# FindoraNetwork/ark-bulletproofs

Hardware: AMD Instinct MI355X
Metric: r1cs_constraints_proved_per_sec (+ r1cs_batch_verifies_per_sec under "verify") (higher is better)
Workload: dtype u32x9 (256-bit modular integers, radix 2^29)

## Files before the change

ark_bulletproofs_amd/csrc/ec.cuh:

```cuda
#pragma once
#include "fp29.cuh"

namespace arkbp {

struct Aff {
    Fe x, y;
};
struct Jac {
    Fe X, Y, Z;
};

ARKBP_HD bool aff_is_inf(const Aff& p) { return fe_is_zero_exact(p.x) && fe_is_zero_exact(p.y); }
ARKBP_HD bool jac_is_inf(const Jac& p) { return fe_is_zero_exact(p.Z); }
template <class C> ARKBP_HD Jac jac_inf() {
    Jac r;
    r.X = fe_one<typename C::Fq>();
    r.Y = fe_one<typename C::Fq>();
    r.Z = fe_zero<typename C::Fq>();
    return r;
}
template <class C> ARKBP_HD Jac jac_from_aff(const Aff& p) {
    if (aff_is_inf(p)) return jac_inf<C>();
    Jac r;
    r.X = p.x;
// ... 51 lines not shown
        o.Y = fe_wred<F>(fe_sub<F, 16>(Y3, fe_times<8>(YYYY)));
        o.Z = fe_mul<F>(fe_dbl(p.Y), p.Z);
    }
    return o;
}

template <class C> ARKBP_HD Jac jac_madd(const Jac& p, const Aff& q) {
    typedef typename C::Fq F;
    if (aff_is_inf(q)) return p;
    if (jac_is_inf(p)) {
        Jac r;
        r.X = q.x;
        r.Y = fe_wred<F>(q.y);
        r.Z = fe_one<F>();
        return r;
    }
    Fe Z1Z1 = fe_sqr<F>(p.Z);
    Fe U2 = fe_mul<F>(q.x, Z1Z1);
    Fe S2 = fe_mul<F>(q.y, fe_mul<F>(p.Z, Z1Z1));
    Fe H = fe_sub<F, 4>(U2, p.X);
    Fe r = fe_sub<F, 4>(S2, p.Y);
    if (fe_is_zero_mod<F>(H)) {
        if (fe_is_zero_mod<F>(r)) return jac_dbl<C>(p);
        return jac_inf<C>();
    }
    Fe HH = fe_sqr<F>(H);
    Fe HHH = fe_mul<F>(H, HH);
    Fe V = fe_mul<F>(p.X, HH);
    Jac o;
    o.X = fe_wred<F>(fe_sub<F, 4>(fe_sqr<F>(r), fe_add(HHH, fe_dbl(V))));
    o.Y = fe_mul2<F>(r, fe_sub<F, 4>(V, o.X), fe_neg<F, 4>(p.Y), HHH);
    o.Z = fe_mul<F>(p.Z, H);
    return o;
}

template <class C> ARKBP_HD Jac jac_madd_fast(const Jac& p, const Aff& q, bool& rare) {
    typedef typename C::Fq F;
    Fe Z1Z1 = fe_sqr<F>(p.Z);
    Fe U2 = fe_mul<F>(q.x, Z1Z1);
    Fe S2 = fe_mul<F>(q.y, fe_mul<F>(p.Z, Z1Z1));
    Fe H = fe_sub<F, 4>(U2, p.X);
    Fe r = fe_sub<F, 4>(S2, p.Y);
    rare = aff_is_inf(q) | jac_is_inf(p) | fe_maybe_zero_mod<F>(H);
    Fe HH = fe_sqr<F>(H);
    Fe HHH = fe_mul<F>(H, HH);
    Fe V = fe_mul<F>(p.X, HH);
    Jac o;
    o.X = fe_wred<F>(fe_sub<F, 4>(fe_sqr<F>(r), fe_add(HHH, fe_dbl(V))));
    o.Y = fe_mul2<F>(r, fe_sub<F, 4>(V, o.X), fe_neg<F, 4>(p.Y), HHH);
    o.Z = fe_mul<F>(p.Z, H);
    return o;
}

template <class C> ARKBP_HD Jac jac_add(const Jac& p, const Jac& q) {
    typedef typename C::Fq F;
    if (jac_is_inf(q)) return p;
    if (jac_is_inf(p)) return q;
    Fe Z1Z1 = fe_sqr<F>(p.Z), Z2Z2 = fe_sqr<F>(q.Z);
    Fe U1 = fe_mul<F>(p.X, Z2Z2), U2 = fe_mul<F>(q.X, Z1Z1);
    Fe S1 = fe_mul<F>(p.Y, fe_mul<F>(q.Z, Z2Z2)), S2 = fe_mul<F>(q.Y, fe_mul<F>(p.Z, Z1Z1));
    Fe H = fe_sub<F, 2>(U2, U1);
    Fe r = fe_sub<F, 2>(S2, S1);
    if (fe_is_zero_mod<F>(H)) {
        if (fe_is_zero_mod<F>(r)) return jac_dbl<C>(p);
        return jac_inf<C>();
    }
    Fe HH = fe_sqr<F>(H);
    Fe HHH = fe_mul<F>(H, HH);
    Fe V = fe_mul<F>(U1, HH);
    Jac o;
    o.X = fe_wred<F>(fe_sub<F, 4>(fe_sqr<F>(r), fe_add(HHH, fe_dbl(V))));
    o.Y = fe_mul2<F>(r, fe_sub<F, 4>(V, o.X), fe_neg<F, 2>(S1), HHH);
    o.Z = fe_mul<F>(fe_mul<F>(p.Z, q.Z), H);
    return o;
}

template <class C> ARKBP_HD Aff jac_to_aff_with_zinv(const Jac& p, const Fe& zinv) {
    typedef typename C::Fq F;
    Aff r;
    if (jac_is_inf(p)) {
        r.x = fe_zero<F>();
        r.y = fe_zero<F>();
        return r;
    }
    Fe zi2 = fe_sqr<F>(zinv);
    r.x = fe_canon<F>(fe_mul<F>(p.X, zi2));
    r.y = fe_canon<F>(fe_mul<F>(p.Y, fe_mul<F>(zi2, zinv)));
    return r;
}
template <class C> ARKBP_HD Aff jac_to_aff(const Jac& p) {
    return jac_to_aff_with_zinv<C>(p, fe_inv<typename C::Fq>(p.Z));
}

template <class F> ARKBP_DEV_NOINLINE bool fe_sqrt(Fe& out, const Fe& a_in) {
    const Fe a = fe_wred<F>(a_in);
    if (fe_is_zero_mod<F>(a)) { out = fe_zero<F>(); return true; }
    const Fe a2 = fe_sqr<F>(a), a3 = fe_mul<F>(a2, a);
    Fe w = fe_one<F>();
#pragma unroll 1
    for (int wd = 7; wd >= 0; wd--) {
        const u32 e = F::TS_TM1H[wd];
#pragma unroll 1
        for (int bit = 30; bit >= 0; bit -= 2) {
            w = fe_sqr<F>(fe_sqr<F>(w));
            const u32 d = (e >> bit) & 3u;
            if (d) {
// ... 83 lines not shown
```

ark_bulletproofs_amd/csrc/fp29.cuh:

```cuda
#pragma once
#include <cstdint>
#if defined(__HIPCC__)
#include <hip/hip_runtime.h>
#define ARKBP_HD __host__ __device__ __forceinline__
#define ARKBP_DEV_NOINLINE __device__ __noinline__
#else
#define ARKBP_HD inline
#define ARKBP_DEV_NOINLINE inline
#endif
#include "arkbp_params.h"

#ifdef ARKBP_CHECK_BOUNDS
#include <cstdio>
#include <cstdlib>
#define ARKBP_ASSERT(c, msg) do { if (!(c)) { fprintf(stderr, "fp29 bound violated: %s (%s:%d)\n", msg, __FILE__, __LINE__); abort(); } } while (0)
#else
#define ARKBP_ASSERT(c, msg)
#endif

namespace arkbp {

typedef uint32_t u32;
typedef uint64_t u64;
typedef int32_t i32;
// ... 61 lines not shown
    static_assert(K == 2 || K == 4 || K == 8 || K == 16, "K");
    Fe r;
#pragma unroll
    for (int i = 0; i < 9; i++) {
        const u32 off = K == 2 ? P::SUBK2[i] : K == 4 ? P::SUBK4[i] : K == 8 ? P::SUBK8[i] : P::SUBK16[i];
        ARKBP_ASSERT(i == 8 || a.l[i] <= (2u << 29), "fe_sub: L(a) > 2");
        ARKBP_ASSERT(b.l[i] <= off, "fe_sub: limb of b exceeds the K*p offset");
        r.l[i] = a.l[i] + off - b.l[i];
    }
    return fe_norm(r);
}
template <class P, int K> ARKBP_HD Fe fe_neg(const Fe& a) { return fe_sub<P, K>(fe_zero<P>(), a); }

template <class P, class Col> ARKBP_HD Fe fe_pm_product(Col&& col) {
    static_assert(P::PM, "pseudo-Mersenne fields only");
    constexpr u32 c0 = P::PM_C0, c1 = P::PM_C1;
    u32 H[9];
    u64 acc = 0;
#pragma unroll
    for (int k = 9; k < 17; k++) {
        col(k, acc);
        H[k - 9] = (u32)acc & M29;
        acc >>= 29;
    }
    ARKBP_ASSERT(acc < (1ull << 32), "fe_pm_product: product exceeds 18 limbs");
    H[8] = (u32)acc;
    Fe r;
    acc = 0;
#pragma unroll
    for (int k = 0; k < 9; k++) {
        col(k, acc);
        acc += (u64)H[k] * c0;
        if (c1 != 0 && k > 0) acc += (u64)H[k - 1] * c1;
        r.l[k] = (u32)acc & M29;
        acc >>= 29;
    }
    if (c1 != 0) acc += (u64)H[8] * c1;
    const u64 o1 = acc;
    ARKBP_ASSERT(o1 < (1ull << 41), "fe_pm_product: overflow too large");
    constexpr int sh = P::BITS - 232;
    const u64 o = (o1 << (261 - P::BITS)) + (r.l[8] >> sh);
    r.l[8] &= (1u << sh) - 1u;
    acc = (u64)r.l[0] + o * P::PM_D0;
    r.l[0] = (u32)acc & M29; acc >>= 29;
    acc += (u64)r.l[1] + o * P::PM_D1;
    r.l[1] = (u32)acc & M29; acc >>= 29;
    u32 cy = (u32)acc;
#pragma unroll
    for (int j = 2; j < 8; j++) { const u32 t = r.l[j] + cy; r.l[j] = t & M29; cy = t >> 29; }
    r.l[8] += cy;
    return r;
}

template <class P> ARKBP_HD Fe fe_mul(const Fe& a, const Fe& b) {
#ifdef ARKBP_CHECK_BOUNDS
    { u64 la = 0, lb = 0; for (int i = 0; i < 9; i++) { if (a.l[i] > la) la = a.l[i]; if (b.l[i] > lb) lb = b.l[i]; }
      ARKBP_ASSERT((unsigned __int128)la * lb <= ((unsigned __int128)6 << 58) + ((unsigned __int128)1 << 40), "fe_mul: L(a)*L(b) > 6"); }
#endif
    if constexpr (P::PM) {
        return fe_pm_product<P>([&](int k, u64& acc) {
#pragma unroll
            for (int i = (k < 9 ? 0 : k - 8); i <= (k < 9 ? k : 8); i++) acc += (u64)a.l[i] * b.l[k - i];
        });
    }
    u32 m[9];
    Fe t;
    u64 acc = 0;
#pragma unroll
    for (int k = 0; k < 9; k++) {
#pragma unroll
        for (int i = 0; i <= k; i++) acc += (u64)a.l[i] * b.l[k - i];
#pragma unroll
        for (int i = 0; i < k; i++) acc += (u64)m[i] * P::P29[k - i];
        m[k] = ((u32)acc * P::NINV29) & M29;
        acc += (u64)m[k] * P::P29[0];
        acc >>= 29;
    }
#pragma unroll
    for (int k = 9; k < 17; k++) {
#pragma unroll
        for (int i = k - 8; i < 9; i++) acc += (u64)a.l[i] * b.l[k - i];
#pragma unroll
        for (int i = k - 8; i < 9; i++) acc += (u64)m[i] * P::P29[k - i];
        t.l[k - 9] = (u32)acc & M29;
        acc >>= 29;
    }
    ARKBP_ASSERT(acc < (1ull << 29), "fe_mul: result exceeds 2^261");
    t.l[8] = (u32)acc;
    return t;
}

template <class P> ARKBP_HD Fe fe_mul2(const Fe& a, const Fe& b, const Fe& c, const Fe& d) {
#ifdef ARKBP_CHECK_BOUNDS
    { u64 la = 0, lb = 0, lc = 0, ld = 0;
      for (int i = 0; i < 9; i++) { if (a.l[i] > la) la = a.l[i]; if (b.l[i] > lb) lb = b.l[i]; if (c.l[i] > lc) lc = c.l[i]; if (d.l[i] > ld) ld = d.l[i]; }
      ARKBP_ASSERT((unsigned __int128)la * lb + (unsigned __int128)lc * ld <= ((unsigned __int128)6 << 58) + ((unsigned __int128)1 << 41), "fe_mul2: L(a)*L(b) + L(c)*L(d) > 6"); }
#endif
    if constexpr (P::PM) {
        return fe_pm_product<P>([&](int k, u64& acc) {
#pragma unroll
            for (int i = (k < 9 ? 0 : k - 8); i <= (k < 9 ? k : 8); i++) { acc += (u64)a.l[i] * b.l[k - i]; acc += (u64)c.l[i] * d.l[k - i]; }
        });
    }
    u32 m[9];
    Fe t;
    u64 acc = 0;
#pragma unroll
    for (int k = 0; k < 9; k++) {
#pragma unroll
        for (int i = 0; i <= k; i++) { acc += (u64)a.l[i] * b.l[k - i]; acc += (u64)c.l[i] * d.l[k - i]; }
#pragma unroll
        for (int i = 0; i < k; i++) acc += (u64)m[i] * P::P29[k - i];
        m[k] = ((u32)acc * P::NINV29) & M29;
        acc += (u64)m[k] * P::P29[0];
        acc >>= 29;
    }
#pragma unroll
    for (int k = 9; k < 17; k++) {
#pragma unroll
        for (int i = k - 8; i < 9; i++) { acc += (u64)a.l[i] * b.l[k - i]; acc += (u64)c.l[i] * d.l[k - i]; }
#pragma unroll
        for (int i = k - 8; i < 9; i++) acc += (u64)m[i] * P::P29[k - i];
        t.l[k - 9] = (u32)acc & M29;
        acc >>= 29;
    }
    ARKBP_ASSERT(acc < (1ull << 29), "fe_mul2: result exceeds 2^261");
    t.l[8] = (u32)acc;
    return t;
}

template <class P> ARKBP_HD Fe fe_sqr(const Fe& a) {
    u32 m[9], a2[9];
#pragma unroll
    for (int i = 0; i < 9; i++) a2[i] = a.l[i] << 1;
#ifdef ARKBP_CHECK_BOUNDS
    for (int i = 0; i < 9; i++) ARKBP_ASSERT(a.l[i] <= (2u << 29) + 16, "fe_sqr: L(a) > 2");
#endif
    if constexpr (P::PM) {
        return fe_pm_product<P>([&](int k, u64& acc) {
#pragma unroll
            for (int i = (k < 9 ? 0 : k - 8); 2 * i < k; i++) acc += (u64)a2[i] * a.l[k - i];
            if ((k & 1) == 0) acc += (u64)a.l[k / 2] * a.l[k / 2];
        });
    }
    Fe t;
    u64 acc = 0;
#pragma unroll
    for (int k = 0; k < 9; k++) {
#pragma unroll
        for (int i = 0; 2 * i < k; i++) acc += (u64)a2[i] * a.l[k - i];
        if ((k & 1) == 0) acc += (u64)a.l[k / 2] * a.l[k / 2];
#pragma unroll
        for (int i = 0; i < k; i++) acc += (u64)m[i] * P::P29[k - i];
        m[k] = ((u32)acc * P::NINV29) & M29;
        acc += (u64)m[k] * P::P29[0];
        acc >>= 29;
    }
#pragma unroll
    for (int k = 9; k < 17; k++) {
#pragma unroll
        for (int i = k - 8; 2 * i < k; i++) acc += (u64)a2[i] * a.l[k - i];
        if ((k & 1) == 0) acc += (u64)a.l[k / 2] * a.l[k / 2];
#pragma unroll
        for (int i = k - 8; i < 9; i++) acc += (u64)m[i] * P::P29[k - i];
        t.l[k - 9] = (u32)acc & M29;
        acc >>= 29;
    }
    t.l[8] = (u32)acc;
    return t;
}

template <class P> ARKBP_HD Fe fe_wred(const Fe& a) {
    if constexpr (P::PM) {
        constexpr int shp = P::BITS - 232;
        ARKBP_ASSERT(a.l[8] < (1u << 29) + 8u, "fe_wred: a >= 2^261");
        const u32 o = a.l[8] >> shp;
        Fe r;
        u32 t = a.l[0] + o * P::PM_D0;
        r.l[0] = t & M29;
        t = a.l[1] + o * P::PM_D1 + (t >> 29);
        r.l[1] = t & M29;
        u32 cy = t >> 29;
#pragma unroll
        for (int j = 2; j < 8; j++) { t = a.l[j] + cy; r.l[j] = t & M29; cy = t >> 29; }
        r.l[8] = (a.l[8] & ((1u << shp) - 1u)) + cy;
        return r;
    }
    constexpr int sh = P::WR_BITS - 232;
    u32 q = a.l[8] >> sh;
    if (P::WR_SIGN > 0) q = q ? q - 1 : 0;
    Fe r;
    i64 acc = 0;
#pragma unroll
    for (int i = 0; i < 9; i++) {
        acc += (i64)a.l[i] - (i64)((u64)q * P::P29[i]);
        r.l[i] = (u32)acc & M29;
        acc >>= 29;
    }
    ARKBP_ASSERT(acc == 0, "fe_wred: went negative or overflowed");
    return r;
}

template <class P> ARKBP_HD Fe fe_canon(const Fe& a) {
    Fe w = fe_wred<P>(a);
#pragma unroll
    for (int rep = 0; rep < 2; rep++) {
        Fe d;
        i32 c = 0;
#pragma unroll
        for (int i = 0; i < 9; i++) {
            i32 t = (i32)w.l[i] - (i32)P::P29[i] + c;
            d.l[i] = (u32)t & M29;
            c = t >> 29;
        }
        const bool neg = c < 0;
#pragma unroll
        for (int i = 0; i < 9; i++) w.l[i] = neg ? w.l[i] : d.l[i];
// ... 80 lines not shown
```

ark_bulletproofs_amd/csrc/ipa.cuh:

```cuda
#pragma once
#include "msm.cuh"

namespace arkbp {

template <class F> __global__ void k_scalars_import(const u32* __restrict__ in, u32* __restrict__ out, u32 n) {
    const u32 i = blockIdx.x * blockDim.x + threadIdx.x;
    if (i >= n) return;
    u32 w[8];
    load_words8(w, in + (size_t)i * 8);
    store_fe_dev<F>(out + (size_t)i * 8, fe_load_ark<F>(w));
}
template <class F> __global__ void k_scalars_export(const u32* __restrict__ in, u32* __restrict__ out, u32 n) {
    const u32 i = blockIdx.x * blockDim.x + threadIdx.x;
    if (i >= n) return;
    u32 w[8];
    fe_store_ark<F>(w, load_fe_dev<F>(in + (size_t)i * 8));
    store_words8(out + (size_t)i * 8, w);
}

static constexpr int IMPORT_MAX = 5;
struct ImportList {
    u32* dst[IMPORT_MAX];
    u32 cnt[IMPORT_MAX];
    int nseg;
// ... 443 lines not shown
        u32 w[16];
        aff_store_dev(w, o);
        store_words8(out + ((size_t)e * n + i) * 16, w);
        store_words8(out + ((size_t)e * n + i) * 16 + 8, w + 8);
    }
}
template <class C> __device__ __forceinline__ bool jac_equals_aff(const Jac& J, const Aff& A) {
    typedef typename C::Fq F;
    const bool ji = jac_is_inf(J), ai = aff_is_inf(A);
    if (ji || ai) return ji && ai;
    const Fe zz = fe_sqr<F>(J.Z);
    if (!fe_eq_mod<F>(fe_wred<F>(J.X), fe_mul<F>(A.x, zz))) return false;
    return fe_eq_mod<F>(fe_wred<F>(J.Y), fe_mul<F>(A.y, fe_mul<F>(zz, J.Z)));
}
template <class C> __global__ void __launch_bounds__(256)
k_ftab_check(const u32* __restrict__ gens, const u32* __restrict__ T, u32 n, u32 E, u32 nwin, unsigned long long* __restrict__ bad,
             u32 g_first = 0, u32 g_stride = 1 ) {
    const u32 i = blockIdx.x * blockDim.x + threadIdx.x;
    if (i >= n) return;
    u32 wrong = 0;
    Aff first = load_aff_dev(gens + ((size_t)g_first + (size_t)i * g_stride) * 16);
    Jac expect = jac_from_aff<C>(first);
#pragma unroll 1
    for (u32 j = 0; j < nwin; j++) {
        const u32* row = T + ((size_t)j * E) * n * 16;
        const Aff base = load_aff_dev(row + (size_t)i * 16);
        if (!jac_equals_aff<C>(expect, base)) wrong++;
        Aff prev = base;
#pragma unroll 1
        for (u32 e = 2; e <= E; e++) {
            const Aff cur = load_aff_dev(row + ((size_t)(e - 1) * n + i) * 16);
            if (!jac_equals_aff<C>(jac_madd<C>(jac_from_aff<C>(prev), base), cur)) wrong++;
            prev = cur;
        }
        expect = jac_dbl<C>(jac_from_aff<C>(prev));
    }
    if (wrong) atomicAdd(bad, (unsigned long long)wrong);
}
template <class C> __global__ void __launch_bounds__(256)
k_fb_rows_check(const u32* __restrict__ gens, const u32* __restrict__ T, u32 n, size_t row_points, u32 R, unsigned long long* __restrict__ bad) {
    const u32 i = blockIdx.x * blockDim.x + threadIdx.x;
    if (i >= n) return;
    u32 wrong = 0;
    Jac expect = jac_from_aff<C>(load_aff_dev(gens + (size_t)i * 16));
#pragma unroll 1
    for (u32 r = 0; r < R; r++) {
        const Aff cur = load_aff_dev(T + ((size_t)r * row_points + i) * 16);
        if (!jac_equals_aff<C>(expect, cur)) wrong++;
        expect = jac_dbl<C>(jac_dbl<C>(jac_dbl<C>(jac_dbl<C>(jac_from_aff<C>(cur)))));
    }
    if (wrong) atomicAdd(bad, (unsigned long long)wrong);
}

template <class C> __device__ __forceinline__ Jac ftab_step(Jac acc, const u32* __restrict__ T, u32 n_tab, u32 E, u32 gi, u32 j, u32 e1, u32 e2, bool neg1, bool neg2) {
    typedef typename C::Fq F;
#pragma unroll 1
    for (int h = 0; h < (C::HAS_GLV ? 2 : 1); h++) {
        const u32 e = h ? e2 : e1;
        if (!e) continue;
        const u32* src = T + (((size_t)j * E + (e - 1)) * n_tab + gi) * 16;
        const bool neg = h ? neg2 : neg1;
        Aff P = load_aff_dev(src);
        if constexpr (C::HAS_GLV) { if (h && !aff_is_inf(P)) P.x = fe_mul<F>(P.x, fe_const<F, C::BETA29>()); }
        bool rare;
        Jac nxt = jac_madd_fast<C>(acc, aff_cneg_lazy<C>(P, neg), rare);
        if (__builtin_expect(rare, 0)) {
            Aff Q = load_aff_dev(src);
            if constexpr (C::HAS_GLV) { if (h && !aff_is_inf(Q)) Q.x = fe_mul<F>(Q.x, fe_const<F, C::BETA29>()); }
            nxt = jac_madd<C>(acc, aff_cneg_lazy<C>(Q, neg));
        }
        acc = nxt;
    }
    return acc;
}
template <class C> __global__ void __launch_bounds__(256) __attribute__((amdgpu_waves_per_eu(3)))
k_ipa_fold_tab(const u32* __restrict__ TG, const u32* __restrict__ TH, u32 n_tab, u32 E, u32* __restrict__ G, u32* __restrict__ H, u32 n, FtabDigits dG,
               FtabDigits dH, int which, u32 g_first, u32 g_stride, u32* __restrict__ jac_ws,
               const u32* __restrict__ Gin ,
               const u32* __restrict__ Hin) {
    typedef typename C::Fq F;
    const u32 t = blockIdx.x * blockDim.x + threadIdx.x;
    if (t >= (which == 3 ? 2 * n : n)) return;
    const bool isH = which == 2 || (which == 3 && t >= n);
    const u32 i = (which == 3 && isH) ? t - n : t;
    u32* V = isH ? H : G;
    const u32* T = isH ? TH : TG;
    const u32 gi = g_first + i * g_stride;
    Jac acc = jac_inf<C>();
    const u32 nwin = isH ? dH.nwin : dG.nwin;
#pragma unroll 1
    for (u32 j = 0; j < nwin; j++) {
        const u32 e1 = isH ? dH.e1[j] : dG.e1[j], e2 = isH ? dH.e2[j] : dG.e2[j];
        acc = ftab_step<C>(acc, T, n_tab, E, gi, j, e1, e2, (((isH ? dH.neg1 : dG.neg1) >> j) & 1ull) != 0, (((isH ? dH.neg2 : dG.neg2) >> j) & 1ull) != 0);
    }
    const u32* Vin = isH ? (Hin ? Hin : H) : (Gin ? Gin : G);
    acc = jac_madd<C>(acc, load_aff_dev(Vin + (size_t)(n + i) * 16));
    fold_emit<C>(V, i, t, acc, jac_ws);
}

struct FtabDigits3 {
    FtabDigits d[3];
};
template <class C> __global__ void __launch_bounds__(256) __attribute__((amdgpu_waves_per_eu(3)))
k_ipa_fold_tab2(const u32* __restrict__ TG, const u32* __restrict__ TH, u32 n_tab, u32 E, u32* __restrict__ G, u32* __restrict__ H, u32 m, FtabDigits3 dG,
                FtabDigits3 dH, u32* __restrict__ jac_ws, const u32* __restrict__ Gin, const u32* __restrict__ Hin,
                u32 g_first , u32 g_stride) {
    typedef typename C::Fq F;
    const u32 t = blockIdx.x * blockDim.x + threadIdx.x;
    if (t >= 2 * m) return;
    const bool isH = t >= m;
    const u32 i = isH ? t - m : t;
    const u32 n = 2 * m;
    const u32* T = isH ? TH : TG;
    Jac acc = jac_inf<C>();
#pragma unroll 1
    for (u32 mu = 0; mu < 3; mu++) {
        const u32 gi = g_first + (mu == 0 ? m + i : mu == 1 ? n + i : i) * g_stride;
        const u32 nwin = isH ? dH.d[mu].nwin : dG.d[mu].nwin;
        const unsigned long long neg1 = isH ? dH.d[mu].neg1 : dG.d[mu].neg1, neg2 = isH ? dH.d[mu].neg2 : dG.d[mu].neg2;
#pragma unroll 1
        for (u32 j = 0; j < nwin; j++) {
            const u32 e1 = isH ? dH.d[mu].e1[j] : dG.d[mu].e1[j], e2 = isH ? dH.d[mu].e2[j] : dG.d[mu].e2[j];
            acc = ftab_step<C>(acc, T, n_tab, E, gi, j, e1, e2, ((neg1 >> j) & 1ull) != 0, ((neg2 >> j) & 1ull) != 0);
        }
    }
    acc = jac_madd<C>(acc, load_aff_dev((isH ? Hin : Gin) + (size_t)(n + m + i) * 16));
    fold_emit<C>(isH ? H : G, i, t, acc, jac_ws);
}

}
```

ark_bulletproofs_amd/csrc/msm.cuh:

```cuda
#pragma once
#include "ec.cuh"
#include "fe_io.cuh"
#include "ecq.cuh"
#include "glv.cuh"

namespace arkbp {

#ifndef ARKBP_MSM_CH
#define ARKBP_MSM_CH 16
#endif
static constexpr int MSM_CH = ARKBP_MSM_CH;
static constexpr int MSM_CHL = MSM_CH == 8 ? 3 : MSM_CH == 16 ? 4 : MSM_CH == 32 ? 5 : 6;
static_assert((1 << MSM_CHL) == MSM_CH, "ARKBP_MSM_CH must be 8, 16, 32 or 64");
static constexpr int MSM_CHL_BINNED = MSM_CHL;
static constexpr int MSM_MAXLVL = 8;
static constexpr int MSM_MAXSEG = 6;

struct BaseSegs {
    const u32* ptr[MSM_MAXSEG];
    u32 start[MSM_MAXSEG + 1];
    int nseg;
    u32 fixed_c4;
    u32 tbits;
    u64 row_words[MSM_MAXSEG];
// ... 452 lines not shown
    for (u32 j = 0; j < 8; j++) {
        const u32 b = base + j;
        if (b >= B) break;
        u32 v = cnt[j];
        for (int k = 0; k < nl; k++) { lvl_off[(size_t)k * (B + 1) + b] = excl[k]; excl[k] += v; v = msm_next_level(v, k, chl, b >= b_gen, spl); }
    }
}

__global__ void __launch_bounds__(256) k_msm_scatter(const u32* __restrict__ canon, u32* __restrict__ cursor, u32* __restrict__ entries, MsmPlan pl) {
    const u32 i = blockIdx.x * blockDim.x + threadIdx.x;
    const bool live = i < pl.n;
    u32 k[8];
#pragma unroll
    for (int j = 0; j < 8; j++) k[j] = 0;
    if (live) load_words8(k, canon + (size_t)i * 8);
    u32 carry = 0;
    for (int w = 0; w < pl.W; w++) {
        const int d = msm_digit(k, w, pl.c, carry);
        const bool valid = live && d != 0 && w >= pl.w_lo && w < pl.w_hi;
        const u32 pos = wave_count(cursor, (u32)w * pl.NB + (u32)(d < 0 ? -d : d) - 1, valid);
        if (valid) entries[pos] = (i << 1) | (d < 0 ? 1u : 0u);
    }
}

__device__ __forceinline__ u32 find_bucket(const u32* __restrict__ off, u32 B, u32 j) {
    u32 lo = 0, hi = B;
    while (hi - lo > 1) {
        u32 mid = (lo + hi) >> 1;
        if (off[mid] <= j) lo = mid; else hi = mid;
    }
    return lo;
}

template <class C> __global__ void __launch_bounds__(256)
k_msm_accum(BaseSegs segs, const u32* __restrict__ entries, const u32* __restrict__ off0, const u32* __restrict__ off1, u32* __restrict__ out,
            u32 B, u32 nchunks, int slotted, SlotPlan sp, u32 NB, const u32* __restrict__ boff, int chl) {
    const u32 j = blockIdx.x * blockDim.x + threadIdx.x;
    if (j >= nchunks) return;
    const u32 b = find_bucket(off1, B, j);
    u32 beg, end;
    const u32 r = j - off1[b], k = off1[b + 1] - off1[b];
    u32 s0, cnt;
    if (slotted == 2) {
        s0 = boff[b]; cnt = off0[b + 1] - off0[b];
    } else if (slotted) {
        const u32 w = b / NB, v = b - w * NB;
        s0 = sp.base[w] + v * sp.cap[w]; cnt = off0[b + 1] - off0[b];
    } else {
        s0 = off0[b]; cnt = off0[b + 1] - off0[b];
    }
    const u32 per = k > 1 ? (cnt + k - 1) / k : (1u << chl);
    beg = s0 + min(r * per, cnt);
    end = min(beg + per, s0 + cnt);
    Jac acc = jac_inf<C>();
    if (beg < end) {
        u32 ent = entries[beg];
        u32 ent_n = beg + 1 < end ? entries[beg + 1] : 0u;
        Raw16 raw = load_raw16(seg_base_ptr(segs, ent >> 1));
        for (u32 e = beg; e < end; e++) {
            Raw16 raw_n = raw;
            u32 ent_nn = 0;
            if (e + 1 < end) raw_n = load_raw16(seg_base_ptr(segs, ent_n >> 1));
            if (e + 2 < end) ent_nn = entries[e + 2];
            const Aff p = aff_from_raw(raw);
            if (e == beg) {
                acc = jac_from_aff<C>(aff_cneg_lazy<C>(p, ent & 1));
                acc.Y = fe_wred<typename C::Fq>(acc.Y);
            } else {
                bool rare;
                Jac nxt = jac_madd_fast<C>(acc, aff_cneg_lazy<C>(p, ent & 1), rare);
                if (__builtin_expect(rare, 0)) nxt = jac_madd<C>(acc, aff_cneg_lazy<C>(load_aff_dev(seg_base_ptr(segs, ent >> 1)), ent & 1));
                acc = nxt;
            }
            ent = ent_n; ent_n = ent_nn;
            raw = raw_n;
        }
    }
    store_jac_ws<C>(out + (size_t)j * 24, acc);
}

template <class C> __global__ void __launch_bounds__(256)
k_msm_accum_wave(BaseSegs segs, const u32* __restrict__ entries, const u32* __restrict__ off0, const u32* __restrict__ off_last, u32* __restrict__ out, u32 B,
                 int slotted, SlotPlan sp, u32 NB, const u32* __restrict__ boff) {
    __shared__ u32 sh[4][64 * 27];
    const u32 wv = threadIdx.x >> 6, lane = threadIdx.x & 63;
    const u32 b = blockIdx.x * 4 + wv;
    if (b >= B) return;
    const u32 cnt = off0[b + 1] - off0[b];
    if (!cnt) return;
    u32 beg;
    if (slotted == 2) beg = boff[b];
    else if (slotted) { const u32 w = b / NB, v = b - w * NB; beg = sp.base[w] + v * sp.cap[w]; }
    else beg = off0[b];
    Jac acc = jac_inf<C>();
    for (u32 e = lane; e < cnt; e += 64) {
        const u32 ent = entries[beg + e];
        acc = jac_madd<C>(acc, aff_cneg_lazy<C>(load_aff_dev(seg_base_ptr(segs, ent >> 1)), ent & 1));
    }
    u32* s = sh[wv];
    for (u32 stride = 32; stride >= 1; stride >>= 1) {
        if (lane >= stride && lane < 2 * stride) {
#pragma unroll
            for (int i = 0; i < 9; i++) { s[i * 64 + lane] = acc.X.l[i]; s[(9 + i) * 64 + lane] = acc.Y.l[i]; s[(18 + i) * 64 + lane] = acc.Z.l[i]; }
        }
        __builtin_amdgcn_wave_barrier();
        __threadfence_block();
        if (lane < stride) {
            Jac o;
#pragma unroll
            for (int i = 0; i < 9; i++) { o.X.l[i] = s[i * 64 + lane + stride]; o.Y.l[i] = s[(9 + i) * 64 + lane + stride]; o.Z.l[i] = s[(18 + i) * 64 + lane + stride]; }
            acc = jac_add<C>(acc, o);
        }
        __builtin_amdgcn_wave_barrier();
        __threadfence_block();
    }
    if (lane == 0) store_jac_ws<C>(out + (size_t)off_last[b] * 24, acc);
}

template <class C> __global__ void __launch_bounds__(256)
k_msm_reduce(const u32* __restrict__ in, const u32* __restrict__ off_prev, const u32* __restrict__ off_cur, u32* __restrict__ out, u32 B,
             u32 nchunks, int chl, u32 skip_from ) {
    const u32 j = blockIdx.x * blockDim.x + threadIdx.x;
    if (j >= nchunks) return;
    const u32 b = find_bucket(off_cur, B, j);
    if (b >= skip_from) return;
    const u32 beg = off_prev[b] + ((j - off_cur[b]) << chl);
    const u32 end = min(beg + (1u << chl), off_prev[b + 1]);
    Jac acc = load_jac_ws(in + (size_t)beg * 24);
    for (u32 e = beg + 1; e < end; e++) acc = jac_add<C>(acc, load_jac_ws(in + (size_t)e * 24));
    store_jac_ws<C>(out + (size_t)j * 24, acc);
}
// ... 237 lines not shown
        if ((int)lane >= o) { incl += t2; inclc += t3; }
    }
    if (lane == 63) { wsum[wv] = incl; wsum[4 + wv] = inclc; }
    __syncthreads();
    u32 excl = incl - run, exclc = inclc - runc;
    for (u32 q = 0; q < wv; q++) { excl += wsum[q]; exclc += wsum[4 + q]; }
    const u32 b0 = w * pl.NB + (bin << bp.LB);
    for (u32 x = tid * per; x < min((tid + 1) * per, NF); x++) {
        const u32 cn = cnt[x];
        bcnt[b0 + x] = cn;
        boff[b0 + x] = (u32)region + excl;
        loff[b0 + x] = exclc;
        cnt[x] = excl;
        excl += cn;
        exclc += (cn + chm) / chcap;
    }
    if (tid == 255) bin_chunks[w * bp.NBIN + bin] = exclc;
    if (big > MSM_FS_BUCKET_MAX) *overflow = 1u;
    __syncthreads();
    for (u32 x = tid; x < n; x += 256) {
        const u32 e = buf[x];
        const u32 pos = atomicAdd(&cnt[(e >> 1) & fmask], 1u);
        ent[region + pos] = ((e >> (bp.LB + 1)) << 1) | (e & 1u);
    }
}
__device__ __forceinline__ void fs_bin_range(u32 x, const MsmPlan& pl, const BinPlan& bp, u32& b0, u32& nb) {
    if (x < bp.wb * bp.NBIN) { const u32 w = x / bp.NBIN, bin = x - w * bp.NBIN; b0 = w * (u32)pl.NB + (bin << bp.LB); nb = 1u << bp.LB; }
    else { b0 = ((u32)pl.W - 1u) * (u32)pl.NB; nb = bp.top_nb; }
}
template <class C> __global__ void __launch_bounds__(256)
k_msm_accum_fs(BaseSegs segs, const u32* __restrict__ entries, const u32* __restrict__ bcnt, const u32* __restrict__ loff, const u32* __restrict__ boff,
               const u32* __restrict__ bin_chunks, u32* __restrict__ out, MsmPlan pl, BinPlan bp, FsPlan fp, u32 chcap, u32* __restrict__ info) {
    __shared__ u32 base[MSM_FS_MAXBINS + 1];
    __shared__ u32 ws[4];
    fs_block_scan(bin_chunks, fp.nbins, base, ws);
    const u32 total = min(base[fp.nbins], fp.max_chunks);
    if (blockIdx.x == 0 && threadIdx.x == 0) { info[0] = base[fp.nbins]; info[1] = base[fp.nbins - 1]; }
    const u32 j = blockIdx.x * 256u + threadIdx.x;
    if (j >= total) return;
    u32 lo = 0, hi = fp.nbins;
    while (hi - lo > 1) { const u32 mid = (lo + hi) >> 1; if (base[mid] <= j) lo = mid; else hi = mid; }
    const u32 jj = j - base[lo];
    u32 b0, nb;
    fs_bin_range(lo, pl, bp, b0, nb);
    u32 l2 = 0, h2 = nb;
    while (h2 - l2 > 1) { const u32 mid = (l2 + h2) >> 1; if (loff[b0 + mid] <= jj) l2 = mid; else h2 = mid; }
    const u32 b = b0 + l2;
    const u32 s0 = boff[b];
    const u32 cnt = bcnt[b], r = jj - loff[b];
    const u32 k = (cnt + chcap - 1u) / chcap;
    const u32 per = k > 1 ? (cnt + k - 1) / k : chcap;
    const u32 beg = s0 + min(r * per, cnt);
    const u32 end = min(beg + per, s0 + cnt);
    Jac acc = jac_inf<C>();
    if (beg < end) {
        u32 ent = entries[beg];
        u32 ent_n = beg + 1 < end ? entries[beg + 1] : 0u;
        Raw16 raw = load_raw16(seg_base_ptr(segs, ent >> 1));
        for (u32 e = beg; e < end; e++) {
            Raw16 raw_n = raw;
            u32 ent_nn = 0;
            if (e + 1 < end) raw_n = load_raw16(seg_base_ptr(segs, ent_n >> 1));
            if (e + 2 < end) ent_nn = entries[e + 2];
            Aff p = aff_from_raw(raw);
            if constexpr (C::HAS_GLV) {
                if (segs.glv && (ent & 2u) && !aff_is_inf(p)) p.x = fe_mul<typename C::Fq>(p.x, fe_const<typename C::Fq, C::BETA29>());
            }
            if (e == beg) {
                acc = jac_from_aff<C>(aff_cneg_lazy<C>(p, ent & 1));
                acc.Y = fe_wred<typename C::Fq>(acc.Y);
            } else {
                bool rare;
                Jac nxt = jac_madd_fast<C>(acc, aff_cneg_lazy<C>(p, ent & 1), rare);
                if (__builtin_expect(rare, 0)) {
                    Aff q = load_aff_dev(seg_base_ptr(segs, ent >> 1));
                    if constexpr (C::HAS_GLV) {
                        if (segs.glv && (ent & 2u) && !aff_is_inf(q)) q.x = fe_mul<typename C::Fq>(q.x, fe_const<typename C::Fq, C::BETA29>());
                    }
                    nxt = jac_madd<C>(acc, aff_cneg_lazy<C>(q, ent & 1));
                }
                acc = nxt;
            }
            ent = ent_n; ent_n = ent_nn;
            raw = raw_n;
        }
    }
    store_jac_ws<C>(out + (size_t)j * 24, acc);
}
template <class C, bool QUAD = false> __global__ void __launch_bounds__(256)
k_msm_reduce_fs(const u32* __restrict__ part, const u32* __restrict__ bcnt, const u32* __restrict__ loff, const u32* __restrict__ bin_chunks,
                u32* __restrict__ sums, MsmPlan pl, BinPlan bp, FsPlan fp, u32 chcap, u32 G) {
    __shared__ u32 base[MSM_FS_MAXBINS + 1];
    __shared__ u32 ws[4];
    fs_block_scan(bin_chunks, fp.nbins, base, ws);
    const u32 g = blockIdx.x * 256u + threadIdx.x;
    const u32 nbk = bp.wb * (u32)pl.NB;
    const u32 gb = G == 4 ? g >> 2 : g;
    const u32 b = min(gb, nbk - 1u), q = G == 4 ? g & 3u : 0u;
    const u32 w = b / (u32)pl.NB, v = b - w * (u32)pl.NB;
    const u32 first = base[w * bp.NBIN + (v >> bp.LB)] + loff[b];
    u32 nch = min((bcnt[b] + chcap - 1u) / chcap, MSM_FS_BUCKET_MAX / 8u);
    if (first + nch > fp.max_chunks) nch = 0;
    if (QUAD) {
        Jac acc = jac_inf<C>();
        if (nch) acc = load_jac_ws(part + (size_t)first * 24);
#pragma unroll 1
        for (u32 e = 1; e < nch; e++) acc = qjac_add<C>(acc, load_jac_ws(part + (size_t)(first + e) * 24), q);
        if (q == 0 && gb < nbk) store_jac_ws<C>(sums + (size_t)b * 24, acc);
        return;
    }
    Jac acc = jac_inf<C>();
    u32 e = q;
    int o = 0;
#pragma unroll 1
    while (o >= 0) {
        Jac other;
        bool doit;
        if (o == 0) {
            doit = e < nch;
            if (!__any(doit)) { o = G == 4 ? 2 : -1; continue; }
            if (doit) other = load_jac_ws(part + (size_t)(first + e) * 24);
            e += G;
        } else {
            other = jac_shfl_down(acc, o, 4);
            doit = (int)q < o && q + (u32)o < nch;
            o = o == 2 ? 1 : -1;
        }
        if (doit) acc = jac_add<C>(acc, other);
    }
    if (q == 0 && gb < nbk) store_jac_ws<C>(sums + (size_t)b * 24, acc);
}
template <class C> __device__ __forceinline__ void store_T_ark(u32* __restrict__ o, const Jac& acc) {
    typedef typename C::Fq F;
    u32 wd[8];
    const bool inf = jac_is_inf(acc);
    fe_store_ark<F>(wd, acc.X); store_words8(o, wd);
    fe_store_ark<F>(wd, acc.Y); store_words8(o + 8, wd);
    if (inf) { for (int i = 0; i < 8; i++) wd[i] = 0; } else fe_store_ark<F>(wd, acc.Z);
    store_words8(o + 16, wd);
}
// ... 119 lines not shown
```

Before: 16.83 million.

## Use XYZZ coordinates for bucket and table accumulation; exploit all-ones modulus limbs

Replaces Jacobian accumulators with XYZZ coordinates in the MSM bucket-accumulate kernels and the fixed-table fold steps. Mixed addition then needs about 8 multiplies instead of about 11, and the result is converted back to Jacobian once at the end. Separately, the Montgomery reduction columns group modulus limbs equal to 2^29-1 so their products are summed first and multiplied once, cutting multiplies for moduli with such limbs. The risks are more live registers from the extra coordinate, which may cut occupancy, and slower rare paths that go through conversions.

```diff
diff --git a/ark_bulletproofs_amd/csrc/ec.cuh b/ark_bulletproofs_amd/csrc/ec.cuh
--- a/ark_bulletproofs_amd/csrc/ec.cuh
+++ b/ark_bulletproofs_amd/csrc/ec.cuh
@@ -127,6 +127,66 @@
     return o;
 }
 
+struct Xyzz {
+    Fe X, Y, ZZ, ZZZ;
+};
+ARKBP_HD bool xyzz_is_inf(const Xyzz& p) { return fe_is_zero_exact(p.ZZ); }
+template <class C> ARKBP_HD Xyzz xyzz_inf() {
+    Xyzz r;
+    r.X = fe_one<typename C::Fq>();
+    r.Y = fe_one<typename C::Fq>();
+    r.ZZ = fe_zero<typename C::Fq>();
+    r.ZZZ = fe_zero<typename C::Fq>();
+    return r;
+}
+template <class C> ARKBP_HD Xyzz xyzz_from_aff(const Aff& q) {
+    typedef typename C::Fq F;
+    if (aff_is_inf(q)) return xyzz_inf<C>();
+    Xyzz r;
+    r.X = q.x;
+    r.Y = fe_wred<F>(q.y);
+    r.ZZ = fe_one<F>();
+    r.ZZZ = fe_one<F>();
+    return r;
+}
+template <class C> ARKBP_HD Xyzz xyzz_from_jac(const Jac& p) {
+    typedef typename C::Fq F;
+    Xyzz r;
+    r.X = p.X;
+    r.Y = p.Y;
+    r.ZZ = fe_sqr<F>(p.Z);
+    r.ZZZ = fe_mul<F>(p.Z, r.ZZ);
+    return r;
+}
+template <class C> ARKBP_HD Jac xyzz_to_jac(const Xyzz& p) {
+    typedef typename C::Fq F;
+    Jac r;
+    r.X = fe_mul<F>(p.X, p.ZZ);
+    r.Y = fe_mul<F>(p.Y, p.ZZZ);
+    r.Z = p.ZZ;
+    return r;
+}
+template <class C> ARKBP_HD Xyzz xyzz_madd_fast(const Xyzz& p, const Aff& q, bool& rare) {
+    typedef typename C::Fq F;
+    Fe U2 = fe_mul<F>(q.x, p.ZZ);
+    Fe S2 = fe_mul<F>(q.y, p.ZZZ);
+    Fe H = fe_sub<F, 4>(U2, p.X);
+    Fe r = fe_sub<F, 4>(S2, p.Y);
+    rare = aff_is_inf(q) | xyzz_is_inf(p) | fe_maybe_zero_mod<F>(H);
+    Fe HH = fe_sqr<F>(H);
+    Fe HHH = fe_mul<F>(H, HH);
+    Fe V = fe_mul<F>(p.X, HH);
+    Xyzz o;
+    o.X = fe_wred<F>(fe_sub<F, 4>(fe_sqr<F>(r), fe_add(HHH, fe_dbl(V))));
+    o.Y = fe_mul2<F>(r, fe_sub<F, 4>(V, o.X), fe_neg<F, 4>(p.Y), HHH);
+    o.ZZ = fe_mul<F>(p.ZZ, HH);
+    o.ZZZ = fe_mul<F>(p.ZZZ, HHH);
+    return o;
+}
+template <class C> ARKBP_HD Xyzz xyzz_madd(const Xyzz& p, const Aff& q) {
+    return xyzz_from_jac<C>(jac_madd<C>(xyzz_to_jac<C>(p), q));
+}
+
 template <class C> ARKBP_HD Jac jac_add(const Jac& p, const Jac& q) {
     typedef typename C::Fq F;
     if (jac_is_inf(q)) return p;
diff --git a/ark_bulletproofs_amd/csrc/fp29.cuh b/ark_bulletproofs_amd/csrc/fp29.cuh
--- a/ark_bulletproofs_amd/csrc/fp29.cuh
+++ b/ark_bulletproofs_amd/csrc/fp29.cuh
@@ -137,6 +137,23 @@
     return r;
 }
 
+template <class P> constexpr int fe_ones_limbs() {
+    int n = 0;
+    for (int i = 0; i < 9; i++) n += P::P29[i] == M29 ? 1 : 0;
+    return n;
+}
+template <class P> ARKBP_HD void fe_red_col(u64& acc, const u32 (&m)[9], int k, int lo, int hi) {
+    static_assert(fe_ones_limbs<P>() <= 7, "the sum of the m[i] under all-ones limbs must fit 32 bits");
+    u32 ones = 0;
+    bool any = false;
+#pragma unroll
+    for (int i = lo; i < hi; i++) {
+        if (P::P29[k - i] == M29) { ones += m[i]; any = true; }
+        else acc += (u64)m[i] * P::P29[k - i];
+    }
+    if (any) acc += (u64)ones * M29;
+}
+
 template <class P> ARKBP_HD Fe fe_mul(const Fe& a, const Fe& b) {
 #ifdef ARKBP_CHECK_BOUNDS
     { u64 la = 0, lb = 0; for (int i = 0; i < 9; i++) { if (a.l[i] > la) la = a.l[i]; if (b.l[i] > lb) lb = b.l[i]; }
@@ -155,8 +172,7 @@
     for (int k = 0; k < 9; k++) {
 #pragma unroll
         for (int i = 0; i <= k; i++) acc += (u64)a.l[i] * b.l[k - i];
-#pragma unroll
-        for (int i = 0; i < k; i++) acc += (u64)m[i] * P::P29[k - i];
+        fe_red_col<P>(acc, m, k, 0, k);
         m[k] = ((u32)acc * P::NINV29) & M29;
         acc += (u64)m[k] * P::P29[0];
         acc >>= 29;
@@ -165,8 +181,7 @@
     for (int k = 9; k < 17; k++) {
 #pragma unroll
         for (int i = k - 8; i < 9; i++) acc += (u64)a.l[i] * b.l[k - i];
-#pragma unroll
-        for (int i = k - 8; i < 9; i++) acc += (u64)m[i] * P::P29[k - i];
+        fe_red_col<P>(acc, m, k, k - 8, 9);
         t.l[k - 9] = (u32)acc & M29;
         acc >>= 29;
     }
@@ -194,8 +209,7 @@
     for (int k = 0; k < 9; k++) {
 #pragma unroll
         for (int i = 0; i <= k; i++) { acc += (u64)a.l[i] * b.l[k - i]; acc += (u64)c.l[i] * d.l[k - i]; }
-#pragma unroll
-        for (int i = 0; i < k; i++) acc += (u64)m[i] * P::P29[k - i];
+        fe_red_col<P>(acc, m, k, 0, k);
         m[k] = ((u32)acc * P::NINV29) & M29;
         acc += (u64)m[k] * P::P29[0];
         acc >>= 29;
@@ -204,8 +218,7 @@
     for (int k = 9; k < 17; k++) {
 #pragma unroll
         for (int i = k - 8; i < 9; i++) { acc += (u64)a.l[i] * b.l[k - i]; acc += (u64)c.l[i] * d.l[k - i]; }
-#pragma unroll
-        for (int i = k - 8; i < 9; i++) acc += (u64)m[i] * P::P29[k - i];
+        fe_red_col<P>(acc, m, k, k - 8, 9);
         t.l[k - 9] = (u32)acc & M29;
         acc >>= 29;
     }
@@ -235,8 +248,7 @@
 #pragma unroll
         for (int i = 0; 2 * i < k; i++) acc += (u64)a2[i] * a.l[k - i];
         if ((k & 1) == 0) acc += (u64)a.l[k / 2] * a.l[k / 2];
-#pragma unroll
-        for (int i = 0; i < k; i++) acc += (u64)m[i] * P::P29[k - i];
+        fe_red_col<P>(acc, m, k, 0, k);
         m[k] = ((u32)acc * P::NINV29) & M29;
         acc += (u64)m[k] * P::P29[0];
         acc >>= 29;
@@ -246,8 +258,7 @@
 #pragma unroll
         for (int i = k - 8; 2 * i < k; i++) acc += (u64)a2[i] * a.l[k - i];
         if ((k & 1) == 0) acc += (u64)a.l[k / 2] * a.l[k / 2];
-#pragma unroll
-        for (int i = k - 8; i < 9; i++) acc += (u64)m[i] * P::P29[k - i];
+        fe_red_col<P>(acc, m, k, k - 8, 9);
         t.l[k - 9] = (u32)acc & M29;
         acc >>= 29;
     }
diff --git a/ark_bulletproofs_amd/csrc/ipa.cuh b/ark_bulletproofs_amd/csrc/ipa.cuh
--- a/ark_bulletproofs_amd/csrc/ipa.cuh
+++ b/ark_bulletproofs_amd/csrc/ipa.cuh
@@ -519,7 +519,7 @@
     if (wrong) atomicAdd(bad, (unsigned long long)wrong);
 }
 
-template <class C> __device__ __forceinline__ Jac ftab_step(Jac acc, const u32* __restrict__ T, u32 n_tab, u32 E, u32 gi, u32 j, u32 e1, u32 e2, bool neg1, bool neg2) {
+template <class C> __device__ __forceinline__ Xyzz ftab_step(Xyzz acc, const u32* __restrict__ T, u32 n_tab, u32 E, u32 gi, u32 j, u32 e1, u32 e2, bool neg1, bool neg2) {
     typedef typename C::Fq F;
 #pragma unroll 1
     for (int h = 0; h < (C::HAS_GLV ? 2 : 1); h++) {
@@ -530,11 +530,11 @@
         Aff P = load_aff_dev(src);
         if constexpr (C::HAS_GLV) { if (h && !aff_is_inf(P)) P.x = fe_mul<F>(P.x, fe_const<F, C::BETA29>()); }
         bool rare;
-        Jac nxt = jac_madd_fast<C>(acc, aff_cneg_lazy<C>(P, neg), rare);
+        Xyzz nxt = xyzz_madd_fast<C>(acc, aff_cneg_lazy<C>(P, neg), rare);
         if (__builtin_expect(rare, 0)) {
             Aff Q = load_aff_dev(src);
             if constexpr (C::HAS_GLV) { if (h && !aff_is_inf(Q)) Q.x = fe_mul<F>(Q.x, fe_const<F, C::BETA29>()); }
-            nxt = jac_madd<C>(acc, aff_cneg_lazy<C>(Q, neg));
+            nxt = xyzz_madd<C>(acc, aff_cneg_lazy<C>(Q, neg));
         }
         acc = nxt;
     }
@@ -553,7 +553,7 @@
     u32* V = isH ? H : G;
     const u32* T = isH ? TH : TG;
     const u32 gi = g_first + i * g_stride;
-    Jac acc = jac_inf<C>();
+    Xyzz acc = xyzz_inf<C>();
     const u32 nwin = isH ? dH.nwin : dG.nwin;
 #pragma unroll 1
     for (u32 j = 0; j < nwin; j++) {
@@ -561,8 +561,7 @@
         acc = ftab_step<C>(acc, T, n_tab, E, gi, j, e1, e2, (((isH ? dH.neg1 : dG.neg1) >> j) & 1ull) != 0, (((isH ? dH.neg2 : dG.neg2) >> j) & 1ull) != 0);
     }
     const u32* Vin = isH ? (Hin ? Hin : H) : (Gin ? Gin : G);
-    acc = jac_madd<C>(acc, load_aff_dev(Vin + (size_t)(n + i) * 16));
-    fold_emit<C>(V, i, t, acc, jac_ws);
+    fold_emit<C>(V, i, t, jac_madd<C>(xyzz_to_jac<C>(acc), load_aff_dev(Vin + (size_t)(n + i) * 16)), jac_ws);
 }
 
 struct FtabDigits3 {
@@ -579,7 +578,7 @@
     const u32 i = isH ? t - m : t;
     const u32 n = 2 * m;
     const u32* T = isH ? TH : TG;
-    Jac acc = jac_inf<C>();
+    Xyzz acc = xyzz_inf<C>();
 #pragma unroll 1
     for (u32 mu = 0; mu < 3; mu++) {
         const u32 gi = g_first + (mu == 0 ? m + i : mu == 1 ? n + i : i) * g_stride;
@@ -591,8 +590,7 @@
             acc = ftab_step<C>(acc, T, n_tab, E, gi, j, e1, e2, ((neg1 >> j) & 1ull) != 0, ((neg2 >> j) & 1ull) != 0);
         }
     }
-    acc = jac_madd<C>(acc, load_aff_dev((isH ? Hin : Gin) + (size_t)(n + m + i) * 16));
-    fold_emit<C>(isH ? H : G, i, t, acc, jac_ws);
-}
-
-}
+    fold_emit<C>(isH ? H : G, i, t, jac_madd<C>(xyzz_to_jac<C>(acc), load_aff_dev((isH ? Hin : Gin) + (size_t)(n + m + i) * 16)), jac_ws);
+}
+
+}
diff --git a/ark_bulletproofs_amd/csrc/msm.cuh b/ark_bulletproofs_amd/csrc/msm.cuh
--- a/ark_bulletproofs_amd/csrc/msm.cuh
+++ b/ark_bulletproofs_amd/csrc/msm.cuh
@@ -528,7 +528,7 @@
     const u32 per = k > 1 ? (cnt + k - 1) / k : (1u << chl);
     beg = s0 + min(r * per, cnt);
     end = min(beg + per, s0 + cnt);
-    Jac acc = jac_inf<C>();
+    Xyzz acc = xyzz_inf<C>();
     if (beg < end) {
         u32 ent = entries[beg];
         u32 ent_n = beg + 1 < end ? entries[beg + 1] : 0u;
@@ -540,19 +540,18 @@
             if (e + 2 < end) ent_nn = entries[e + 2];
             const Aff p = aff_from_raw(raw);
             if (e == beg) {
-                acc = jac_from_aff<C>(aff_cneg_lazy<C>(p, ent & 1));
-                acc.Y = fe_wred<typename C::Fq>(acc.Y);
+                acc = xyzz_from_aff<C>(aff_cneg_lazy<C>(p, ent & 1));
             } else {
                 bool rare;
-                Jac nxt = jac_madd_fast<C>(acc, aff_cneg_lazy<C>(p, ent & 1), rare);
-                if (__builtin_expect(rare, 0)) nxt = jac_madd<C>(acc, aff_cneg_lazy<C>(load_aff_dev(seg_base_ptr(segs, ent >> 1)), ent & 1));
+                Xyzz nxt = xyzz_madd_fast<C>(acc, aff_cneg_lazy<C>(p, ent & 1), rare);
+                if (__builtin_expect(rare, 0)) nxt = xyzz_madd<C>(acc, aff_cneg_lazy<C>(load_aff_dev(seg_base_ptr(segs, ent >> 1)), ent & 1));
                 acc = nxt;
             }
             ent = ent_n; ent_n = ent_nn;
             raw = raw_n;
         }
     }
-    store_jac_ws<C>(out + (size_t)j * 24, acc);
+    store_jac_ws<C>(out + (size_t)j * 24, xyzz_to_jac<C>(acc));
 }
 
 template <class C> __global__ void __launch_bounds__(256)
@@ -896,7 +895,7 @@
     const u32 per = k > 1 ? (cnt + k - 1) / k : chcap;
     const u32 beg = s0 + min(r * per, cnt);
     const u32 end = min(beg + per, s0 + cnt);
-    Jac acc = jac_inf<C>();
+    Xyzz acc = xyzz_inf<C>();
     if (beg < end) {
         u32 ent = entries[beg];
         u32 ent_n = beg + 1 < end ? entries[beg + 1] : 0u;
@@ -911,17 +910,16 @@
                 if (segs.glv && (ent & 2u) && !aff_is_inf(p)) p.x = fe_mul<typename C::Fq>(p.x, fe_const<typename C::Fq, C::BETA29>());
             }
             if (e == beg) {
-                acc = jac_from_aff<C>(aff_cneg_lazy<C>(p, ent & 1));
-                acc.Y = fe_wred<typename C::Fq>(acc.Y);
+                acc = xyzz_from_aff<C>(aff_cneg_lazy<C>(p, ent & 1));
             } else {
                 bool rare;
-                Jac nxt = jac_madd_fast<C>(acc, aff_cneg_lazy<C>(p, ent & 1), rare);
+                Xyzz nxt = xyzz_madd_fast<C>(acc, aff_cneg_lazy<C>(p, ent & 1), rare);
                 if (__builtin_expect(rare, 0)) {
                     Aff q = load_aff_dev(seg_base_ptr(segs, ent >> 1));
                     if constexpr (C::HAS_GLV) {
                         if (segs.glv && (ent & 2u) && !aff_is_inf(q)) q.x = fe_mul<typename C::Fq>(q.x, fe_const<typename C::Fq, C::BETA29>());
                     }
-                    nxt = jac_madd<C>(acc, aff_cneg_lazy<C>(q, ent & 1));
+                    nxt = xyzz_madd<C>(acc, aff_cneg_lazy<C>(q, ent & 1));
                 }
                 acc = nxt;
             }
@@ -929,7 +927,7 @@
             raw = raw_n;
         }
     }
-    store_jac_ws<C>(out + (size_t)j * 24, acc);
+    store_jac_ws<C>(out + (size_t)j * 24, xyzz_to_jac<C>(acc));
 }
 template <class C, bool QUAD = false> __global__ void __launch_bounds__(256)
 k_msm_reduce_fs(const u32* __restrict__ part, const u32* __restrict__ bcnt, const u32* __restrict__ loff, const u32* __restrict__ bin_chunks,
diff --git a/ark_bulletproofs_amd/csrc/xyzz_selftest.cpp b/ark_bulletproofs_amd/csrc/xyzz_selftest.cpp
--- /dev/null
+++ b/ark_bulletproofs_amd/csrc/xyzz_selftest.cpp
@@ -0,0 +1,54 @@
+#include "ec.cuh"
+using namespace arkbp;
+
+static Fe ld(const u32* w) { Fe r; for (int i = 0; i < 9; i++) r.l[i] = w[i]; return r; }
+static void st(u32* w, const Fe& a) { for (int i = 0; i < 9; i++) w[i] = a.l[i]; }
+static Xyzz ld_xyzz(const u32* w) { Xyzz r; r.X = ld(w); r.Y = ld(w + 9); r.ZZ = ld(w + 18); r.ZZZ = ld(w + 27); return r; }
+static void st_xyzz(u32* w, const Xyzz& p) { st(w, p.X); st(w + 9, p.Y); st(w + 18, p.ZZ); st(w + 27, p.ZZZ); }
+static Jac ld_jac(const u32* w) { Jac r; r.X = ld(w); r.Y = ld(w + 9); r.Z = ld(w + 18); return r; }
+static void st_jac(u32* w, const Jac& p) { st(w, p.X); st(w + 9, p.Y); st(w + 18, p.Z); }
+static Aff ld_aff(const u32* w) { Aff r; r.x = ld(w); r.y = ld(w + 9); return r; }
+
+template <class C> static int madd(int op, const u32* acc36, const u32* q18, int neg, u32* out36) {
+    const Xyzz acc = ld_xyzz(acc36);
+    const Aff q = aff_cneg_lazy<C>(ld_aff(q18), neg != 0);
+    bool rare;
+    Xyzz nxt = xyzz_madd_fast<C>(acc, q, rare);
+    if (op == 1 && rare) nxt = xyzz_madd<C>(acc, q);
+    st_xyzz(out36, nxt);
+    return rare ? 1 : 0;
+}
+template <class C> static void chain(int n, const u32* q18s, const u32* negs, u32* out36s, u32* rares) {
+    Xyzz acc = xyzz_inf<C>();
+    for (int e = 0; e < n; e++) {
+        const Aff q = aff_cneg_lazy<C>(ld_aff(q18s + (size_t)e * 18), negs[e] != 0);
+        if (e == 0) { acc = xyzz_from_aff<C>(q); rares[e] = 0; }
+        else {
+            bool rare;
+            Xyzz nxt = xyzz_madd_fast<C>(acc, q, rare);
+            if (rare) nxt = xyzz_madd<C>(acc, q);
+            rares[e] = rare ? 1 : 0;
+            acc = nxt;
+        }
+        st_xyzz(out36s + (size_t)e * 36, acc);
+    }
+}
+
+extern "C" {
+int xyzz_madd_raw(int cid, int op, const u32* acc36, const u32* q18, int neg, u32* out36) {
+    return cid == 0 ? madd<Secq>(op, acc36, q18, neg, out36) : madd<Zorro>(op, acc36, q18, neg, out36);
+}
+void xyzz_chain_raw(int cid, int n, const u32* q18s, const u32* negs, u32* out36s, u32* rares) {
+    if (cid == 0) chain<Secq>(n, q18s, negs, out36s, rares); else chain<Zorro>(n, q18s, negs, out36s, rares);
+}
+void xyzz_from_jac_raw(int cid, const u32* in27, u32* out36) {
+    st_xyzz(out36, cid == 0 ? xyzz_from_jac<Secq>(ld_jac(in27)) : xyzz_from_jac<Zorro>(ld_jac(in27)));
+}
+void xyzz_to_jac_raw(int cid, const u32* in36, u32* out27) {
+    st_jac(out27, cid == 0 ? xyzz_to_jac<Secq>(ld_xyzz(in36)) : xyzz_to_jac<Zorro>(ld_xyzz(in36)));
+}
+void xyzz_from_aff_raw(int cid, const u32* q18, int neg, u32* out36) {
+    const Aff q = ld_aff(q18);
+    st_xyzz(out36, cid == 0 ? xyzz_from_aff<Secq>(aff_cneg_lazy<Secq>(q, neg != 0)) : xyzz_from_aff<Zorro>(aff_cneg_lazy<Zorro>(q, neg != 0)));
+}
+}
```

Result: slower. 16.64 million (-1.1%).
